# CFSAN-Biostatistics/snp-pipeline

Measured on AMD Instinct MI355X. Metric: consensus_bases_called_per_sec, higher is better.
Workload: dtype u8; 1 GPU; BASELINE configs[3] shard (125 samples/GPU x 5000000 bp x 30x synthetic pileups, 49878 SNP sites, 1500 SNP records per sample; the reference bundles no pileups); step = site-record gather + site union, one batched scan launch + one call launch, 4-bit pack, row all-gather, all-pairs distance tiles, row-band exchange; samples_total=125, samples_this_rank=125, genome_bp=5000000, snp_sites=49878, pileup_bytes_this_rank=54061520755, parallelism=samples sharded over 1 rank(s)

## Files before the change

snp_pipeline_amd/csrc/regions.hip:

```cpp
#include <string.h>

#include <vector>

#include "internal.h"
#include "prims.h"

namespace {

inline size_t up256(size_t x) { return (x + 255) / 256 * 256; }
inline unsigned nblk(uint64_t n) { return (unsigned)((n + 255) / 256); }

#define R_TRY(ctx, expr)                                                                                \
    do {                                                                                                \
        hipError_t e_ = (expr);                                                                         \
        if (e_ != hipSuccess)                                                                           \
            return snpgpu_set_error((ctx), SNPGPU_E_HIP, "%s failed: %s", #expr, hipGetErrorString(e_)); \
    } while (0)

#define REG_ERR_POSITION 1u
#define REG_ERR_INTERVAL 2u

struct U64Less { __device__ bool operator()(const uint64_t &a, const uint64_t &b) const { return a < b; } };

#define MAX_RULES 64
struct Rules { int32_t max_snps[MAX_RULES], window[MAX_RULES]; uint32_t n; };

__device__ __forceinline__ uint32_t seg_of(const uint32_t *seg_off, uint32_t n_segs, uint32_t i) {
    uint32_t lo = 0, hi = n_segs;
    while (hi - lo > 1) { uint32_t mid = (lo + hi) >> 1; if (seg_off[mid] <= i) lo = mid; else hi = mid; }
    return lo;
}

__global__ void k_seg_keys(const int64_t *pos, const uint32_t *seg_off, uint32_t n_segs, uint32_t n_pos, uint64_t *keys, uint32_t *out_n) {
    uint32_t i = blockIdx.x * blockDim.x + threadIdx.x;
    if (i >= n_pos) return;
    int64_t p = pos[i];
    if (p < 0 || p >= (1ll << 40)) { atomicOr(&out_n[1], REG_ERR_POSITION); p = 0; }
    keys[i] = ((uint64_t)seg_of(seg_off, n_segs, i) << 40) | (uint64_t)p;
}

__global__ void k_dense_flags(const uint64_t *keys, const uint32_t *seg_off, uint32_t n_segs, uint32_t n_pos, Rules rules, uint32_t *flag) {
    uint64_t g = (uint64_t)blockIdx.x * blockDim.x + threadIdx.x;
    if (g >= (uint64_t)n_pos * rules.n) return;
    const uint32_t i = (uint32_t)(g / rules.n), r = (uint32_t)(g % rules.n);
    const uint32_t end = seg_off[seg_of(seg_off, n_segs, i) + 1];
    const int64_t m = rules.max_snps[r], mask = (1ll << 40) - 1;
    uint32_t f = 0;
    if (m >= 0 && (uint64_t)i + (uint64_t)m < end) f = ((int64_t)(keys[i] & mask) + (int64_t)rules.window[r] - 1 >= (int64_t)(keys[i + m] & mask)) ? 1u : 0u;
    flag[g] = f;
}

__global__ void k_dense_emit(const uint64_t *keys, uint32_t n_pos, Rules rules, const uint32_t *flag, const uint32_t *slot,
                             int64_t *out_start, int64_t *out_end, uint32_t *out_seg) {
    uint64_t g = (uint64_t)blockIdx.x * blockDim.x + threadIdx.x;
    if (g >= (uint64_t)n_pos * rules.n || !flag[g]) return;
    const uint32_t i = (uint32_t)(g / rules.n), r = (uint32_t)(g % rules.n);
    const uint64_t mask = (1ull << 40) - 1;
    const uint32_t o = slot[g];
    out_start[o] = (int64_t)(keys[i] & mask);
    out_end[o] = (int64_t)(keys[i + rules.max_snps[r]] & mask);
    out_seg[o] = (uint32_t)(keys[i] >> 40);
}

__global__ void k_copy_word(const uint32_t *src, uint32_t *dst) { *dst = *src; }

size_t dense_ws_bytes(uint32_t n_pos, uint32_t n_rules) {
    const uint64_t total = (uint64_t)n_pos * n_rules;
    return 3 * up256(8ull * n_pos) + 256 + 2 * up256(4 * total) + up256(4 * prim_scan_workspace_words(total)) + 256;
}

int dense_enqueue(snpgpu_ctx *ctx, const int64_t *d_pos, const uint32_t *d_seg_off, uint32_t n_segs, uint32_t n_pos, const Rules &rules,
                  int64_t *d_out_start, int64_t *d_out_end, uint32_t *d_out_seg, uint32_t *d_out_n, char *ws) {
    hipStream_t st = ctx->stream;
    const uint64_t total = (uint64_t)n_pos * rules.n;
    size_t o = 0;
    uint64_t *keys = (uint64_t *)(ws + o); o += up256(8ull * n_pos);
    uint64_t *ka = (uint64_t *)(ws + o); o += up256(8ull * n_pos);
    uint64_t *kb = (uint64_t *)(ws + o); o += up256(8ull * n_pos);
    uint32_t *sflag = (uint32_t *)(ws + o); o += 256;
    uint32_t *flag = (uint32_t *)(ws + o); o += up256(4 * total);
    uint32_t *slot = (uint32_t *)(ws + o); o += up256(4 * total);
    uint32_t *scan_ws = (uint32_t *)(ws + o);
    R_TRY(ctx, hipMemsetAsync(d_out_n, 0, 8, st));
    if (n_pos && rules.n) {
        k_seg_keys<<<nblk(n_pos), 256, 0, st>>>(d_pos, d_seg_off, n_segs, n_pos, keys, d_out_n);
        const uint64_t *sorted = prim_sort<uint64_t, U64Less>(st, keys, ka, kb, n_pos, sflag, U64Less());
        k_dense_flags<<<nblk(total), 256, 0, st>>>(sorted, d_seg_off, n_segs, n_pos, rules, flag);
        uint32_t *d_total = nullptr;
        prim_exclusive_scan_u32(st, flag, slot, total, scan_ws, &d_total);
        k_dense_emit<<<nblk(total), 256, 0, st>>>(sorted, n_pos, rules, flag, slot, d_out_start, d_out_end, d_out_seg);
        k_copy_word<<<1, 1, 0, st>>>(d_total, d_out_n);
    }
    R_TRY(ctx, hipGetLastError());
    return SNPGPU_OK;
}

int make_rules(snpgpu_ctx *ctx, const int32_t *max_snps, const int32_t *window, uint32_t n_rules, Rules &rules) {
    if (n_rules > MAX_RULES) return snpgpu_set_error(ctx, SNPGPU_E_UNSUPPORTED, "more than %d dense-window rules", MAX_RULES);
    if (n_rules && (!max_snps || !window)) return snpgpu_set_error(ctx, SNPGPU_E_ARG, "null dense-window argument");
    memset(&rules, 0, sizeof rules);
    rules.n = n_rules;
    for (uint32_t r = 0; r < n_rules; ++r) { rules.max_snps[r] = max_snps[r]; rules.window[r] = window[r]; }
    return SNPGPU_OK;
}

struct Ival { uint32_t group, pad; int64_t start, end; };
struct IvalLess {
    __device__ bool operator()(const Ival &a, const Ival &b) const {
        if (a.group != b.group) return a.group < b.group;
        if (a.start != b.start) return a.start < b.start;
        return a.end < b.end;
    }
};
struct GroupMax { int64_t maxend; uint32_t group, pad; };
struct GroupMaxOp {
    __device__ GroupMax operator()(const GroupMax &a, const GroupMax &b) const {
        GroupMax r;
        r.group = b.group; r.pad = 0;
        r.maxend = (a.group == b.group && a.maxend > b.maxend) ? a.maxend : b.maxend;
        return r;
    }
};

__global__ void k_ival_pack(const uint32_t *group, const int64_t *start, const int64_t *end, uint32_t n, Ival *out, uint32_t *out_n) {
    uint32_t i = blockIdx.x * blockDim.x + threadIdx.x;
    if (i >= n) return;
    Ival v;
    v.group = group[i]; v.pad = 0; v.start = start[i]; v.end = end[i];
    if (v.start > v.end) atomicOr(&out_n[1], REG_ERR_INTERVAL);
    out[i] = v;
}

__global__ void k_ival_ends(const Ival *sorted, uint32_t n, GroupMax *gm) {
    uint32_t i = blockIdx.x * blockDim.x + threadIdx.x;
    if (i < n) { GroupMax g; g.group = sorted[i].group; g.pad = 0; g.maxend = sorted[i].end; gm[i] = g; }
}

__global__ void k_ival_heads(const Ival *sorted, const GroupMax *run, uint32_t n, uint32_t *head) {
    uint32_t i = blockIdx.x * blockDim.x + threadIdx.x;
    if (i >= n) return;
    uint32_t h = 1;
    if (i > 0 && run[i - 1].group == sorted[i].group) {
        const int64_t le = run[i - 1].maxend;
        h = (le == INT64_MAX || sorted[i].start <= le + 1) ? 0u : 1u;
    }
    head[i] = h;
}

__global__ void k_ival_emit(const Ival *sorted, const GroupMax *run, const uint32_t *head, const uint32_t *slot, uint32_t n,
                            uint32_t *out_group, int64_t *out_start, int64_t *out_end) {
    uint32_t i = blockIdx.x * blockDim.x + threadIdx.x;
    if (i >= n) return;
    const uint32_t o = slot[i] + head[i] - 1;
    if (head[i]) { out_group[o] = sorted[i].group; out_start[o] = sorted[i].start; }
    if (i + 1 == n || head[i + 1]) out_end[o] = run[i].maxend;
}

size_t merge_regions_ws_bytes(uint32_t n) {
    return 3 * up256(sizeof(Ival) * (size_t)n) + 256 + 2 * up256(sizeof(GroupMax) * (size_t)n) + up256(sizeof(GroupMax) * (size_t)prim_gscan_blocks(n)) +
           2 * up256(4ull * n) + up256(4 * prim_scan_workspace_words(n)) + 256;
}

int merge_regions_enqueue(snpgpu_ctx *ctx, const uint32_t *d_group, const int64_t *d_start, const int64_t *d_end, uint32_t n,
                          uint32_t *d_out_group, int64_t *d_out_start, int64_t *d_out_end, uint32_t *d_out_n, char *ws) {
    hipStream_t st = ctx->stream;
    size_t o = 0;
    Ival *iv = (Ival *)(ws + o); o += up256(sizeof(Ival) * (size_t)n);
    Ival *ia = (Ival *)(ws + o); o += up256(sizeof(Ival) * (size_t)n);
    Ival *ib = (Ival *)(ws + o); o += up256(sizeof(Ival) * (size_t)n);
    uint32_t *sflag = (uint32_t *)(ws + o); o += 256;
    GroupMax *gm = (GroupMax *)(ws + o); o += up256(sizeof(GroupMax) * (size_t)n);
    GroupMax *run = (GroupMax *)(ws + o); o += up256(sizeof(GroupMax) * (size_t)n);
    GroupMax *aggr = (GroupMax *)(ws + o); o += up256(sizeof(GroupMax) * (size_t)prim_gscan_blocks(n));
    uint32_t *head = (uint32_t *)(ws + o); o += up256(4ull * n);
    uint32_t *slot = (uint32_t *)(ws + o); o += up256(4ull * n);
    uint32_t *scan_ws = (uint32_t *)(ws + o);
    R_TRY(ctx, hipMemsetAsync(d_out_n, 0, 8, st));
    if (n) {
        k_ival_pack<<<nblk(n), 256, 0, st>>>(d_group, d_start, d_end, n, iv, d_out_n);
        const Ival *sorted = prim_sort<Ival, IvalLess>(st, iv, ia, ib, n, sflag, IvalLess());
        k_ival_ends<<<nblk(n), 256, 0, st>>>(sorted, n, gm);
        prim_inclusive_scan<GroupMax, GroupMaxOp>(st, gm, run, n, aggr, GroupMaxOp());
        k_ival_heads<<<nblk(n), 256, 0, st>>>(sorted, run, n, head);
        uint32_t *d_total = nullptr;
        prim_exclusive_scan_u32(st, head, slot, n, scan_ws, &d_total);
        k_ival_emit<<<nblk(n), 256, 0, st>>>(sorted, run, head, slot, n, d_out_group, d_out_start, d_out_end);
        k_copy_word<<<1, 1, 0, st>>>(d_total, d_out_n);
    }
    R_TRY(ctx, hipGetLastError());
    return SNPGPU_OK;
}

__global__ void k_in_regions(const uint32_t *pos_group, const int64_t *pos, uint32_t n, const uint32_t *reg_off,
                             const int64_t *rs, const int64_t *re, uint32_t n_groups, uint8_t *out) {
    uint32_t i = blockIdx.x * blockDim.x + threadIdx.x;
    if (i >= n) return;
    uint32_t g = pos_group[i];
    uint8_t f = 0;
    if (g < n_groups) {
        int64_t p = pos[i];
        uint32_t lo = reg_off[g], hi = reg_off[g + 1];
        while (lo < hi) {
            uint32_t mid = (lo + hi) >> 1;
            if (rs[mid] <= p) lo = mid + 1; else hi = mid;
        }
        if (lo > reg_off[g]) f = re[lo - 1] >= p;
    }
    out[i] = f;
}

struct Pair { uint64_t key; uint32_t samp, pad; };
struct PairLess {
    __device__ bool operator()(const Pair &a, const Pair &b) const { return a.key != b.key ? a.key < b.key : a.samp < b.samp; }
};

__global__ void k_pair_pack(const uint64_t *keys, const uint32_t *samp, uint32_t n, Pair *out) {
    uint32_t i = blockIdx.x * blockDim.x + threadIdx.x;
    if (i < n) { Pair p; p.key = keys[i]; p.samp = samp[i]; p.pad = 0; out[i] = p; }
}

__global__ void k_sites_flags(const Pair *sorted, uint32_t n, uint32_t *new_key, uint32_t *new_pair) {
    uint32_t i = blockIdx.x * blockDim.x + threadIdx.x;
    if (i >= n) return;
    const bool nk = i == 0 || sorted[i].key != sorted[i - 1].key;
    new_key[i] = nk;
    new_pair[i] = nk || sorted[i].samp != sorted[i - 1].samp;
}

__global__ void k_sites_emit(const Pair *sorted, uint32_t n, const uint32_t *new_key, const uint32_t *new_pair, const uint32_t *key_slot,
                             const uint32_t *pair_slot, const uint32_t *n_keys, const uint32_t *n_pairs, uint64_t *out_unique,
                             uint32_t *out_off, uint32_t *out_carrier, uint32_t *out_n) {
    uint32_t i = blockIdx.x * blockDim.x + threadIdx.x;
    if (i == 0) { out_n[0] = *n_keys; out_n[1] = *n_pairs; out_off[*n_keys] = *n_pairs; }
    if (i >= n) return;
    if (new_pair[i]) out_carrier[pair_slot[i]] = sorted[i].samp;
    if (new_key[i]) { out_unique[key_slot[i]] = sorted[i].key; out_off[key_slot[i]] = pair_slot[i]; }
}

size_t merge_sites_ws_bytes(uint32_t n) {
    return 3 * up256(sizeof(Pair) * (size_t)n) + 256 + 4 * up256(4ull * n) + 2 * up256(4 * prim_scan_workspace_words(n)) + 256;
}

int merge_sites_enqueue(snpgpu_ctx *ctx, const uint64_t *d_keys, const uint32_t *d_samp, uint32_t n, uint64_t *d_out_unique,
                        uint32_t *d_out_off, uint32_t *d_out_carrier, uint32_t *d_out_n, char *ws) {
    hipStream_t st = ctx->stream;
    size_t o = 0;
    Pair *pr = (Pair *)(ws + o); o += up256(sizeof(Pair) * (size_t)n);
    Pair *pa = (Pair *)(ws + o); o += up256(sizeof(Pair) * (size_t)n);
    Pair *pb = (Pair *)(ws + o); o += up256(sizeof(Pair) * (size_t)n);
    uint32_t *sflag = (uint32_t *)(ws + o); o += 256;
    uint32_t *nk = (uint32_t *)(ws + o); o += up256(4ull * n);
    uint32_t *np = (uint32_t *)(ws + o); o += up256(4ull * n);
    uint32_t *ks = (uint32_t *)(ws + o); o += up256(4ull * n);
    uint32_t *ps = (uint32_t *)(ws + o); o += up256(4ull * n);
    uint32_t *scan1 = (uint32_t *)(ws + o); o += up256(4 * prim_scan_workspace_words(n));
    uint32_t *scan2 = (uint32_t *)(ws + o);
    R_TRY(ctx, hipMemsetAsync(d_out_n, 0, 8, st));
    R_TRY(ctx, hipMemsetAsync(d_out_off, 0, 4, st));
    if (n) {
        k_pair_pack<<<nblk(n), 256, 0, st>>>(d_keys, d_samp, n, pr);
        const Pair *sorted = prim_sort<Pair, PairLess>(st, pr, pa, pb, n, sflag, PairLess());
        k_sites_flags<<<nblk(n), 256, 0, st>>>(sorted, n, nk, np);
        uint32_t *t_keys = nullptr, *t_pairs = nullptr;
        prim_exclusive_scan_u32(st, nk, ks, n, scan1, &t_keys);
        prim_exclusive_scan_u32(st, np, ps, n, scan2, &t_pairs);
        k_sites_emit<<<nblk(n), 256, 0, st>>>(sorted, n, nk, np, ks, ps, t_keys, t_pairs, d_out_unique, d_out_off, d_out_carrier, d_out_n);
    }
    R_TRY(ctx, hipGetLastError());
    return SNPGPU_OK;
}

int region_error(snpgpu_ctx *ctx, uint32_t bits) {
    if (bits & REG_ERR_POSITION) return snpgpu_set_error(ctx, SNPGPU_E_UNSUPPORTED, "SNP position outside [0, 2^40)");
    if (bits & REG_ERR_INTERVAL) return snpgpu_set_error(ctx, SNPGPU_E_UNSUPPORTED, "interval with start > end");
    return SNPGPU_OK;
}

}

extern "C" {

int snpgpu_dense_windows_dev(snpgpu_ctx *ctx, const int64_t *d_positions, const uint32_t *d_seg_off, uint32_t n_segs, uint32_t n_pos,
                             const int32_t *max_snps, const int32_t *window, uint32_t n_rules, int64_t *d_out_start,
                             int64_t *d_out_end, uint32_t *d_out_seg, uint32_t *d_out_n) {
    if (!ctx || !d_out_n) return SNPGPU_E_ARG;
    Rules rules;
    int rc = make_rules(ctx, max_snps, window, n_rules, rules);
    if (rc) return rc;
    if ((uint64_t)n_pos * n_rules > 0x7FFFFFFFull) return snpgpu_set_error(ctx, SNPGPU_E_UNSUPPORTED, "too many (position, rule) pairs");
    if (n_segs >= (1u << 24)) return snpgpu_set_error(ctx, SNPGPU_E_UNSUPPORTED, "too many segments");
    if (n_pos && (!d_positions || !d_seg_off || !d_out_start || !d_out_end || !d_out_seg)) return snpgpu_set_error(ctx, SNPGPU_E_ARG, "null dense-window argument");
    R_TRY(ctx, snpgpu_enter(ctx));
    void *ws = nullptr;
    rc = snpgpu_scratch(ctx, dense_ws_bytes(n_pos, n_rules), &ws);
    if (rc) return rc;
    return dense_enqueue(ctx, d_positions, d_seg_off, n_segs, n_pos, rules, d_out_start, d_out_end, d_out_seg, d_out_n, (char *)ws);
}

int snpgpu_merge_regions_dev(snpgpu_ctx *ctx, const uint32_t *d_group, const int64_t *d_start, const int64_t *d_end, uint32_t n,
                             uint32_t *d_out_group, int64_t *d_out_start, int64_t *d_out_end, uint32_t *d_out_n) {
    if (!ctx || !d_out_n) return SNPGPU_E_ARG;
    if (n && (!d_group || !d_start || !d_end || !d_out_group || !d_out_start || !d_out_end)) return snpgpu_set_error(ctx, SNPGPU_E_ARG, "null merge argument");
    R_TRY(ctx, snpgpu_enter(ctx));
    void *ws = nullptr;
    int rc = snpgpu_scratch(ctx, merge_regions_ws_bytes(n), &ws);
    if (rc) return rc;
    return merge_regions_enqueue(ctx, d_group, d_start, d_end, n, d_out_group, d_out_start, d_out_end, d_out_n, (char *)ws);
}

int snpgpu_in_regions_dev(snpgpu_ctx *ctx, const uint32_t *d_pos_group, const int64_t *d_positions, uint32_t n_pos,
                          const uint32_t *d_reg_off, const int64_t *d_reg_start, const int64_t *d_reg_end, uint32_t n_groups,
                          uint8_t *d_out_flag) {
    if (!ctx) return SNPGPU_E_ARG;
    if (n_pos == 0) return SNPGPU_OK;
    if (!d_pos_group || !d_positions || !d_out_flag || (n_groups && !d_reg_off)) return snpgpu_set_error(ctx, SNPGPU_E_ARG, "null in_regions argument");
    R_TRY(ctx, snpgpu_enter(ctx));
    k_in_regions<<<nblk(n_pos), 256, 0, ctx->stream>>>(d_pos_group, d_positions, n_pos, d_reg_off, d_reg_start, d_reg_end, n_groups, d_out_flag);
    R_TRY(ctx, hipGetLastError());
    return SNPGPU_OK;
}

int snpgpu_merge_sites_dev(snpgpu_ctx *ctx, const uint64_t *d_keys, const uint32_t *d_sample_of_key, uint32_t n,
                           uint64_t *d_out_unique, uint32_t *d_out_off, uint32_t *d_out_carrier, uint32_t *d_out_n) {
    if (!ctx || !d_out_n || !d_out_off) return SNPGPU_E_ARG;
    if (n > 0x7FFFFFFFu) return snpgpu_set_error(ctx, SNPGPU_E_UNSUPPORTED, "too many site records");
    if (n && (!d_keys || !d_sample_of_key || !d_out_unique || !d_out_carrier)) return snpgpu_set_error(ctx, SNPGPU_E_ARG, "null merge_sites argument");
    R_TRY(ctx, snpgpu_enter(ctx));
    void *ws = nullptr;
    int rc = snpgpu_scratch(ctx, merge_sites_ws_bytes(n), &ws);
    if (rc) return rc;
    return merge_sites_enqueue(ctx, d_keys, d_sample_of_key, n, d_out_unique, d_out_off, d_out_carrier, d_out_n, (char *)ws);
}

int snpgpu_dense_windows(snpgpu_ctx *ctx, const int64_t *positions, const uint32_t *seg_off, uint32_t n_segs,
                         const int32_t *max_snps, const int32_t *window, uint32_t n_rules,
                         int64_t *out_start, int64_t *out_end, uint32_t *out_seg, uint32_t *out_n) {
    if (!ctx || !out_n) return SNPGPU_E_ARG;
    *out_n = 0;
    if (n_segs == 0 || n_rules == 0) return SNPGPU_OK;
    if (!seg_off) return snpgpu_set_error(ctx, SNPGPU_E_ARG, "null dense-window argument");
    const uint32_t n_pos = seg_off[n_segs];
    if (n_pos == 0) return SNPGPU_OK;
    if (!positions || !out_start || !out_end || !out_seg) return snpgpu_set_error(ctx, SNPGPU_E_ARG, "null dense-window argument");
    Rules rules;
    int rc = make_rules(ctx, max_snps, window, n_rules, rules);
    if (rc) return rc;
    const uint64_t total = (uint64_t)n_pos * n_rules;
    if (total > 0x7FFFFFFFull) return snpgpu_set_error(ctx, SNPGPU_E_UNSUPPORTED, "too many (position, rule) pairs");
    if (n_segs >= (1u << 24)) return snpgpu_set_error(ctx, SNPGPU_E_UNSUPPORTED, "too many segments");
    R_TRY(ctx, snpgpu_enter(ctx));
    hipStream_t st = ctx->stream;
    size_t o = 0;
    const size_t o_pos = o; o += up256(8ull * n_pos);
    const size_t o_seg = o; o += up256(4ull * (n_segs + 1));
    const size_t o_os = o; o += up256(8 * total);
    const size_t o_oe = o; o += up256(8 * total);
    const size_t o_og = o; o += up256(4 * total);
    const size_t o_n = o; o += 256;
    const size_t o_ws = o; o += dense_ws_bytes(n_pos, n_rules);
    void *scr = nullptr;
    rc = snpgpu_scratch(ctx, o, &scr);
    if (rc) return rc;
    char *b = (char *)scr;
    R_TRY(ctx, hipMemcpyAsync(b + o_pos, positions, 8ull * n_pos, hipMemcpyHostToDevice, st));
    R_TRY(ctx, hipMemcpyAsync(b + o_seg, seg_off, 4ull * (n_segs + 1), hipMemcpyHostToDevice, st));
    rc = dense_enqueue(ctx, (const int64_t *)(b + o_pos), (const uint32_t *)(b + o_seg), n_segs, n_pos, rules, (int64_t *)(b + o_os),
                       (int64_t *)(b + o_oe), (uint32_t *)(b + o_og), (uint32_t *)(b + o_n), b + o_ws);
    if (rc) return rc;
    uint32_t res[2] = {0, 0};
    R_TRY(ctx, hipMemcpyAsync(res, b + o_n, 8, hipMemcpyDeviceToHost, st));
    R_TRY(ctx, hipStreamSynchronize(st));
    if (res[1]) return region_error(ctx, res[1]);
    if (res[0]) {
        R_TRY(ctx, hipMemcpyAsync(out_start, b + o_os, 8ull * res[0], hipMemcpyDeviceToHost, st));
        R_TRY(ctx, hipMemcpyAsync(out_end, b + o_oe, 8ull * res[0], hipMemcpyDeviceToHost, st));
        R_TRY(ctx, hipMemcpyAsync(out_seg, b + o_og, 4ull * res[0], hipMemcpyDeviceToHost, st));
        R_TRY(ctx, hipStreamSynchronize(st));
    }
    *out_n = res[0];
    return SNPGPU_OK;
}

int snpgpu_merge_regions(snpgpu_ctx *ctx, const uint32_t *group, const int64_t *start, const int64_t *end,
                         uint32_t n, uint32_t *out_group, int64_t *out_start, int64_t *out_end, uint32_t *out_n) {
    if (!ctx || !out_n) return SNPGPU_E_ARG;
    *out_n = 0;
    if (n == 0) return SNPGPU_OK;
    if (!group || !start || !end || !out_group || !out_start || !out_end) return snpgpu_set_error(ctx, SNPGPU_E_ARG, "null merge argument");
    R_TRY(ctx, snpgpu_enter(ctx));
    hipStream_t st = ctx->stream;
    size_t o = 0;
    const size_t o_g = o; o += up256(4ull * n);
    const size_t o_s = o; o += up256(8ull * n);
    const size_t o_e = o; o += up256(8ull * n);
    const size_t o_og = o; o += up256(4ull * n);
    const size_t o_os = o; o += up256(8ull * n);
    const size_t o_oe = o; o += up256(8ull * n);
    const size_t o_n = o; o += 256;
    const size_t o_ws = o; o += merge_regions_ws_bytes(n);
    void *scr = nullptr;
    int rc = snpgpu_scratch(ctx, o, &scr);
    if (rc) return rc;
    char *b = (char *)scr;
    R_TRY(ctx, hipMemcpyAsync(b + o_g, group, 4ull * n, hipMemcpyHostToDevice, st));
    R_TRY(ctx, hipMemcpyAsync(b + o_s, start, 8ull * n, hipMemcpyHostToDevice, st));
    R_TRY(ctx, hipMemcpyAsync(b + o_e, end, 8ull * n, hipMemcpyHostToDevice, st));
    rc = merge_regions_enqueue(ctx, (const uint32_t *)(b + o_g), (const int64_t *)(b + o_s), (const int64_t *)(b + o_e), n,
                               (uint32_t *)(b + o_og), (int64_t *)(b + o_os), (int64_t *)(b + o_oe), (uint32_t *)(b + o_n), b + o_ws);
    if (rc) return rc;
    uint32_t res[2] = {0, 0};
    R_TRY(ctx, hipMemcpyAsync(res, b + o_n, 8, hipMemcpyDeviceToHost, st));
    R_TRY(ctx, hipStreamSynchronize(st));
    if (res[1]) return region_error(ctx, res[1]);
    R_TRY(ctx, hipMemcpyAsync(out_group, b + o_og, 4ull * res[0], hipMemcpyDeviceToHost, st));
    R_TRY(ctx, hipMemcpyAsync(out_start, b + o_os, 8ull * res[0], hipMemcpyDeviceToHost, st));
    R_TRY(ctx, hipMemcpyAsync(out_end, b + o_oe, 8ull * res[0], hipMemcpyDeviceToHost, st));
    R_TRY(ctx, hipStreamSynchronize(st));
    *out_n = res[0];
    return SNPGPU_OK;
}

int snpgpu_in_regions(snpgpu_ctx *ctx, const uint32_t *pos_group, const int64_t *positions, uint32_t n_pos,
                      const uint32_t *reg_off, const int64_t *reg_start, const int64_t *reg_end,
                      uint32_t n_groups, uint8_t *out_flag) {
    if (!ctx) return SNPGPU_E_ARG;
    if (n_pos == 0) return SNPGPU_OK;
    if (!pos_group || !positions || !out_flag || (n_groups && !reg_off)) return snpgpu_set_error(ctx, SNPGPU_E_ARG, "null in_regions argument");
    R_TRY(ctx, snpgpu_enter(ctx));
    hipStream_t st = ctx->stream;
    const uint32_t n_reg = n_groups ? reg_off[n_groups] : 0;
    size_t o = 0;
    const size_t o_g = o; o += up256(4ull * n_pos);
    const size_t o_p = o; o += up256(8ull * n_pos);
    const size_t o_off = o; o += up256(4ull * (n_groups + 1));
    const size_t o_rs = o; o += up256(8ull * n_reg);
    const size_t o_re = o; o += up256(8ull * n_reg);
    const size_t o_out = o; o += up256(n_pos);
    void *scr = nullptr;
    int rc = snpgpu_scratch(ctx, o + 256, &scr);
    if (rc) return rc;
    char *b = (char *)scr;
    R_TRY(ctx, hipMemcpyAsync(b + o_g, pos_group, 4ull * n_pos, hipMemcpyHostToDevice, st));
    R_TRY(ctx, hipMemcpyAsync(b + o_p, positions, 8ull * n_pos, hipMemcpyHostToDevice, st));
    if (n_groups) R_TRY(ctx, hipMemcpyAsync(b + o_off, reg_off, 4ull * (n_groups + 1), hipMemcpyHostToDevice, st));
    if (n_reg) {
        R_TRY(ctx, hipMemcpyAsync(b + o_rs, reg_start, 8ull * n_reg, hipMemcpyHostToDevice, st));
        R_TRY(ctx, hipMemcpyAsync(b + o_re, reg_end, 8ull * n_reg, hipMemcpyHostToDevice, st));
    }
    k_in_regions<<<nblk(n_pos), 256, 0, st>>>((const uint32_t *)(b + o_g), (const int64_t *)(b + o_p), n_pos, (const uint32_t *)(b + o_off),
                                              (const int64_t *)(b + o_rs), (const int64_t *)(b + o_re), n_groups, (uint8_t *)(b + o_out));
    R_TRY(ctx, hipMemcpyAsync(out_flag, b + o_out, n_pos, hipMemcpyDeviceToHost, st));
    R_TRY(ctx, hipStreamSynchronize(st));
    return SNPGPU_OK;
}

int snpgpu_merge_sites(snpgpu_ctx *ctx, const uint64_t *keys, const uint32_t *sample_of_key, size_t n,
                       uint64_t *out_unique, uint32_t *out_off, uint32_t *out_carrier,
                       uint32_t *out_n_unique, uint32_t *out_n_carrier) {
    if (!ctx || !out_n_unique || !out_n_carrier) return SNPGPU_E_ARG;
    *out_n_unique = *out_n_carrier = 0;
    if (out_off) out_off[0] = 0;
    if (n == 0) return SNPGPU_OK;
    if (n > 0x7FFFFFFFull) return snpgpu_set_error(ctx, SNPGPU_E_UNSUPPORTED, "too many site records");
    if (!keys || !sample_of_key || !out_unique || !out_off || !out_carrier) return snpgpu_set_error(ctx, SNPGPU_E_ARG, "null merge_sites argument");
    R_TRY(ctx, snpgpu_enter(ctx));
    hipStream_t st = ctx->stream;
    const uint32_t m = (uint32_t)n;
    size_t o = 0;
    const size_t o_k = o; o += up256(8ull * m);
    const size_t o_s = o; o += up256(4ull * m);
    const size_t o_u = o; o += up256(8ull * m);
    const size_t o_off = o; o += up256(4ull * (m + 1));
    const size_t o_c = o; o += up256(4ull * m);
    const size_t o_n = o; o += 256;
    const size_t o_ws = o; o += merge_sites_ws_bytes(m);
    void *scr = nullptr;
    int rc = snpgpu_scratch(ctx, o, &scr);
    if (rc) return rc;
    char *b = (char *)scr;
    R_TRY(ctx, hipMemcpyAsync(b + o_k, keys, 8ull * m, hipMemcpyHostToDevice, st));
    R_TRY(ctx, hipMemcpyAsync(b + o_s, sample_of_key, 4ull * m, hipMemcpyHostToDevice, st));
    rc = merge_sites_enqueue(ctx, (const uint64_t *)(b + o_k), (const uint32_t *)(b + o_s), m, (uint64_t *)(b + o_u), (uint32_t *)(b + o_off),
                             (uint32_t *)(b + o_c), (uint32_t *)(b + o_n), b + o_ws);
    if (rc) return rc;
    uint32_t res[2] = {0, 0};
    R_TRY(ctx, hipMemcpyAsync(res, b + o_n, 8, hipMemcpyDeviceToHost, st));
    R_TRY(ctx, hipStreamSynchronize(st));
    R_TRY(ctx, hipMemcpyAsync(out_unique, b + o_u, 8ull * res[0], hipMemcpyDeviceToHost, st));
    R_TRY(ctx, hipMemcpyAsync(out_off, b + o_off, 4ull * (res[0] + 1), hipMemcpyDeviceToHost, st));
    R_TRY(ctx, hipMemcpyAsync(out_carrier, b + o_c, 4ull * res[1], hipMemcpyDeviceToHost, st));
    R_TRY(ctx, hipStreamSynchronize(st));
    *out_n_unique = res[0];
    *out_n_carrier = res[1];
    return SNPGPU_OK;
}

}
```

Baseline: 688.6 million bases/s.

## Replace generic sort and dual scans in site merge with bitonic tiles and merge-path passes

Swaps the generic prim_sort plus two exclusive scans in site-union merging for a purpose-built pipeline. Each 2048-element tile is bitonic-sorted in shared memory, then merge-path passes double the run length. The new-key and new-pair flags are packed into one word so a single count/scan pass (last-block decoupled via a ticket) and one emit pass replace the separate flag, scan and emit kernels. This cuts kernel launches, intermediate buffers and workspace, but packing counts into 16 bits per field limits per-block counts, which holds since blocks are 1024 items.

```diff
diff --git a/snp_pipeline_amd/csrc/regions.hip b/snp_pipeline_amd/csrc/regions.hip
--- a/snp_pipeline_amd/csrc/regions.hip
+++ b/snp_pipeline_amd/csrc/regions.hip
@@ -209,63 +209,183 @@
     out[i] = f;
 }
 
-struct Pair { uint64_t key; uint32_t samp, pad; };
-struct PairLess {
-    __device__ bool operator()(const Pair &a, const Pair &b) const { return a.key != b.key ? a.key < b.key : a.samp < b.samp; }
-};
-
-__global__ void k_pair_pack(const uint64_t *keys, const uint32_t *samp, uint32_t n, Pair *out) {
-    uint32_t i = blockIdx.x * blockDim.x + threadIdx.x;
-    if (i < n) { Pair p; p.key = keys[i]; p.samp = samp[i]; p.pad = 0; out[i] = p; }
-}
-
-__global__ void k_sites_flags(const Pair *sorted, uint32_t n, uint32_t *new_key, uint32_t *new_pair) {
-    uint32_t i = blockIdx.x * blockDim.x + threadIdx.x;
-    if (i >= n) return;
-    const bool nk = i == 0 || sorted[i].key != sorted[i - 1].key;
-    new_key[i] = nk;
-    new_pair[i] = nk || sorted[i].samp != sorted[i - 1].samp;
-}
-
-__global__ void k_sites_emit(const Pair *sorted, uint32_t n, const uint32_t *new_key, const uint32_t *new_pair, const uint32_t *key_slot,
-                             const uint32_t *pair_slot, const uint32_t *n_keys, const uint32_t *n_pairs, uint64_t *out_unique,
-                             uint32_t *out_off, uint32_t *out_carrier, uint32_t *out_n) {
-    uint32_t i = blockIdx.x * blockDim.x + threadIdx.x;
-    if (i == 0) { out_n[0] = *n_keys; out_n[1] = *n_pairs; out_off[*n_keys] = *n_pairs; }
-    if (i >= n) return;
-    if (new_pair[i]) out_carrier[pair_slot[i]] = sorted[i].samp;
-    if (new_key[i]) { out_unique[key_slot[i]] = sorted[i].key; out_off[key_slot[i]] = pair_slot[i]; }
+#define MS_TILE 2048
+#define MS_THREADS 1024
+#define MS_ITEMS 1
+#define MS_BLOCK (MS_THREADS * MS_ITEMS)
+
+struct alignas(16) SitePair { uint64_t key; uint32_t samp, pad; };
+__device__ __forceinline__ bool sp_less(const SitePair &a, const SitePair &b) { return a.key != b.key ? a.key < b.key : a.samp < b.samp; }
+
+inline unsigned ms_tiles(uint32_t n) { return (n + MS_TILE - 1) / MS_TILE; }
+inline unsigned ms_blocks(uint32_t n) { return (n + MS_BLOCK - 1) / MS_BLOCK; }
+
+__global__ __launch_bounds__(MS_THREADS) void k_ms_tiles(const uint64_t *keys, const uint32_t *samp, uint32_t n, SitePair *out, uint32_t *ticket) {
+    __shared__ SitePair tile[MS_TILE];
+    if (blockIdx.x == 0 && threadIdx.x == 0) *ticket = 0;
+    const uint32_t base = blockIdx.x * MS_TILE;
+    const uint32_t cnt = n - base < MS_TILE ? n - base : MS_TILE;
+    for (uint32_t i = threadIdx.x; i < MS_TILE; i += MS_THREADS) {
+        SitePair p;
+        p.key = i < cnt ? keys[base + i] : ~0ull;
+        p.samp = i < cnt ? samp[base + i] : ~0u;
+        p.pad = 0;
+        tile[i] = p;
+    }
+    __syncthreads();
+    for (uint32_t k = 2; k <= MS_TILE; k <<= 1)
+        for (uint32_t j = k >> 1; j > 0; j >>= 1) {
+            for (uint32_t t = threadIdx.x; t < MS_TILE / 2; t += MS_THREADS) {
+                const uint32_t lo = ((t & ~(j - 1)) << 1) | (t & (j - 1)), hi = lo | j;
+                const SitePair a = tile[lo], b = tile[hi];
+                if ((lo & k) == 0 ? sp_less(b, a) : sp_less(a, b)) { tile[lo] = b; tile[hi] = a; }
+            }
+            __syncthreads();
+        }
+    for (uint32_t i = threadIdx.x; i < cnt; i += MS_THREADS) out[base + i] = tile[i];
+}
+
+__global__ __launch_bounds__(MS_THREADS) void k_ms_merge(const SitePair *in, SitePair *out, uint32_t n, uint64_t run) {
+    __shared__ SitePair stage[MS_TILE];
+    __shared__ uint64_t split[2];
+    const uint64_t o0 = (uint64_t)blockIdx.x * MS_TILE;
+    const uint64_t pair0 = o0 / (2 * run) * (2 * run);
+    const uint64_t a_len = n - pair0 < run ? n - pair0 : run;
+    const uint64_t b_begin = pair0 + a_len, b_len = n - b_begin < run ? n - b_begin : run;
+    const uint64_t d0 = o0 - pair0, total = a_len + b_len;
+    const uint64_t d1 = d0 + MS_TILE < total ? d0 + MS_TILE : total;
+    const SitePair *A = in + pair0, *B = in + b_begin;
+    if (threadIdx.x < 128) {
+        const uint32_t lane = threadIdx.x & 63, w = threadIdx.x >> 6;
+        const uint64_t d = w ? d1 : d0;
+        uint64_t lo = d > b_len ? d - b_len : 0, hi = d < a_len ? d : a_len;
+        while (lo < hi) {
+            const uint64_t m = hi - lo;
+            const uint64_t p = m <= 64 ? lo + lane : lo + m * (lane + 1) / 65;
+            const bool first = p < hi && !sp_less(B[d - 1 - p], A[p]);
+            const uint32_t c = (uint32_t)__popcll(__ballot(first));
+            if (m <= 64) { lo += c; hi = lo; }
+            else {
+                const uint64_t nlo = c ? lo + m * c / 65 + 1 : lo;
+                hi = c < 64 ? lo + m * (c + 1) / 65 : hi;
+                lo = nlo;
+            }
+        }
+        if (lane == 0) split[w] = lo;
+    }
+    __syncthreads();
+    const uint64_t a0 = split[0], a1 = split[1], b0 = d0 - a0, b1 = d1 - a1;
+    const uint32_t na = (uint32_t)(a1 - a0), nb = (uint32_t)(b1 - b0);
+    for (uint32_t i = threadIdx.x; i < na + nb; i += MS_THREADS) stage[i] = i < na ? A[a0 + i] : B[b0 + (i - na)];
+    __syncthreads();
+    for (uint32_t i = threadIdx.x; i < na + nb; i += MS_THREADS) {
+        const SitePair v = stage[i];
+        uint32_t lo = 0, hi;
+        if (i < na) {
+            hi = nb;
+            while (lo < hi) { const uint32_t mid = (lo + hi) >> 1; if (sp_less(stage[na + mid], v)) lo = mid + 1; else hi = mid; }
+            out[o0 + i + lo] = v;
+        } else {
+            hi = na;
+            while (lo < hi) { const uint32_t mid = (lo + hi) >> 1; if (!sp_less(v, stage[mid])) lo = mid + 1; else hi = mid; }
+            out[o0 + (i - na) + lo] = v;
+        }
+    }
+}
+
+__device__ __forceinline__ uint32_t ms_flags(const SitePair &prev, const SitePair &cur, bool first) {
+    const bool nk = first || cur.key != prev.key;
+    return (nk ? 0x10000u : 0u) | ((nk || cur.samp != prev.samp) ? 1u : 0u);
+}
+
+__device__ __forceinline__ bool ms_load(const SitePair *sorted, uint32_t n, SitePair (&v)[MS_ITEMS], uint32_t (&f)[MS_ITEMS], uint32_t &sum) {
+    const uint64_t base = (uint64_t)blockIdx.x * MS_BLOCK + (uint64_t)threadIdx.x * MS_ITEMS;
+    sum = 0;
+    if (base >= n) return false;
+    SitePair prev = base ? sorted[base - 1] : SitePair();
+#pragma unroll
+    for (int k = 0; k < MS_ITEMS; ++k) {
+        f[k] = 0;
+        if (base + k < n) { v[k] = sorted[base + k]; f[k] = ms_flags(prev, v[k], base + k == 0); prev = v[k]; }
+        sum += f[k];
+    }
+    return true;
+}
+
+__global__ __launch_bounds__(MS_THREADS) void k_ms_count(const SitePair *sorted, uint32_t n, uint2 *blk, uint32_t *ticket,
+                                                         uint32_t *out_off, uint32_t *out_n) {
+    __shared__ uint32_t lds[17];
+    __shared__ bool last;
+    SitePair v[MS_ITEMS];
+    uint32_t f[MS_ITEMS], s, total;
+    (void)ms_load(sorted, n, v, f, s);
+    (void)block_exclusive_sum(s, lds, total);
+    if (threadIdx.x == 0) {
+        blk[blockIdx.x] = make_uint2(total >> 16, total & 0xFFFFu);
+        __threadfence();
+        last = atomicAdd(ticket, 1u) == gridDim.x - 1;
+    }
+    __syncthreads();
+    if (!last) return;
+    __threadfence();
+    uint32_t ck = 0, cp = 0;
+    for (uint32_t b0 = 0; b0 < gridDim.x; b0 += MS_THREADS) {
+        const uint32_t i = b0 + threadIdx.x;
+        const uint2 c = i < gridDim.x ? blk[i] : make_uint2(0u, 0u);
+        uint32_t tk, tp;
+        const uint32_t ek = block_exclusive_sum(c.x, lds, tk);
+        __syncthreads();
+        const uint32_t ep = block_exclusive_sum(c.y, lds, tp);
+        if (i < gridDim.x) blk[i] = make_uint2(ck + ek, cp + ep);
+        ck += tk; cp += tp;
+        __syncthreads();
+    }
+    if (threadIdx.x == 0) { out_n[0] = ck; out_n[1] = cp; out_off[ck] = cp; }
+}
+
+__global__ __launch_bounds__(MS_THREADS) void k_ms_emit(const SitePair *sorted, uint32_t n, const uint2 *blk, uint64_t *out_unique,
+                                                        uint32_t *out_off, uint32_t *out_carrier) {
+    __shared__ uint32_t lds[17];
+    SitePair v[MS_ITEMS];
+    uint32_t f[MS_ITEMS], s, total;
+    const bool any = ms_load(sorted, n, v, f, s);
+    const uint32_t ex = block_exclusive_sum(s, lds, total);
+    if (!any) return;
+    const uint2 b = blk[blockIdx.x];
+    uint32_t ks = b.x + (ex >> 16), ps = b.y + (ex & 0xFFFFu);
+#pragma unroll
+    for (int k = 0; k < MS_ITEMS; ++k) {
+        if (f[k] & 1u) out_carrier[ps] = v[k].samp;
+        if (f[k] >> 16) { out_unique[ks] = v[k].key; out_off[ks] = ps; }
+        ks += f[k] >> 16; ps += f[k] & 1u;
+    }
 }
 
 size_t merge_sites_ws_bytes(uint32_t n) {
-    return 3 * up256(sizeof(Pair) * (size_t)n) + 256 + 4 * up256(4ull * n) + 2 * up256(4 * prim_scan_workspace_words(n)) + 256;
+    return 2 * up256(sizeof(SitePair) * (size_t)n) + up256(sizeof(uint2) * (size_t)ms_blocks(n)) + 256;
 }
 
 int merge_sites_enqueue(snpgpu_ctx *ctx, const uint64_t *d_keys, const uint32_t *d_samp, uint32_t n, uint64_t *d_out_unique,
                         uint32_t *d_out_off, uint32_t *d_out_carrier, uint32_t *d_out_n, char *ws) {
     hipStream_t st = ctx->stream;
+    if (n == 0) {
+        R_TRY(ctx, hipMemsetAsync(d_out_n, 0, 8, st));
+        R_TRY(ctx, hipMemsetAsync(d_out_off, 0, 4, st));
+        return SNPGPU_OK;
+    }
     size_t o = 0;
-    Pair *pr = (Pair *)(ws + o); o += up256(sizeof(Pair) * (size_t)n);
-    Pair *pa = (Pair *)(ws + o); o += up256(sizeof(Pair) * (size_t)n);
-    Pair *pb = (Pair *)(ws + o); o += up256(sizeof(Pair) * (size_t)n);
-    uint32_t *sflag = (uint32_t *)(ws + o); o += 256;
-    uint32_t *nk = (uint32_t *)(ws + o); o += up256(4ull * n);
-    uint32_t *np = (uint32_t *)(ws + o); o += up256(4ull * n);
-    uint32_t *ks = (uint32_t *)(ws + o); o += up256(4ull * n);
-    uint32_t *ps = (uint32_t *)(ws + o); o += up256(4ull * n);
-    uint32_t *scan1 = (uint32_t *)(ws + o); o += up256(4 * prim_scan_workspace_words(n));
-    uint32_t *scan2 = (uint32_t *)(ws + o);
-    R_TRY(ctx, hipMemsetAsync(d_out_n, 0, 8, st));
-    R_TRY(ctx, hipMemsetAsync(d_out_off, 0, 4, st));
-    if (n) {
-        k_pair_pack<<<nblk(n), 256, 0, st>>>(d_keys, d_samp, n, pr);
-        const Pair *sorted = prim_sort<Pair, PairLess>(st, pr, pa, pb, n, sflag, PairLess());
-        k_sites_flags<<<nblk(n), 256, 0, st>>>(sorted, n, nk, np);
-        uint32_t *t_keys = nullptr, *t_pairs = nullptr;
-        prim_exclusive_scan_u32(st, nk, ks, n, scan1, &t_keys);
-        prim_exclusive_scan_u32(st, np, ps, n, scan2, &t_pairs);
-        k_sites_emit<<<nblk(n), 256, 0, st>>>(sorted, n, nk, np, ks, ps, t_keys, t_pairs, d_out_unique, d_out_off, d_out_carrier, d_out_n);
-    }
+    SitePair *pa = (SitePair *)(ws + o); o += up256(sizeof(SitePair) * (size_t)n);
+    SitePair *pb = (SitePair *)(ws + o); o += up256(sizeof(SitePair) * (size_t)n);
+    uint2 *blk = (uint2 *)(ws + o); o += up256(sizeof(uint2) * (size_t)ms_blocks(n));
+    uint32_t *ticket = (uint32_t *)(ws + o);
+    k_ms_tiles<<<ms_tiles(n), MS_THREADS, 0, st>>>(d_keys, d_samp, n, pa, ticket);
+    SitePair *src = pa, *dst = pb;
+    for (uint64_t run = MS_TILE; run < n; run <<= 1) {
+        k_ms_merge<<<ms_tiles(n), MS_THREADS, 0, st>>>(src, dst, n, run);
+        SitePair *t = src; src = dst; dst = t;
+    }
+    k_ms_count<<<ms_blocks(n), MS_THREADS, 0, st>>>(src, n, blk, ticket, d_out_off, d_out_n);
+    k_ms_emit<<<ms_blocks(n), MS_THREADS, 0, st>>>(src, n, blk, d_out_unique, d_out_off, d_out_carrier);
     R_TRY(ctx, hipGetLastError());
     return SNPGPU_OK;
 }
```

Measured after the change: 700.1 million bases/s (median of 6 runs). 1.7% higher.
